# bupt-ai-cz/HIAST

Measured on AMD Instinct MI355X. Metric: self-training images/sec (fwd+bwd+pseudo-label) at 1024x512, higher is better.
Workload: dtype fp16

## Files before the change

### hiast_amd/_lib.py

```python
import ctypes
import os

import torch

_HERE = os.path.dirname(os.path.abspath(__file__))
LIB_PATH = os.environ.get("HIAST_LIB") or os.path.join(_HERE, "csrc", "libhiast_hip.so")

c_int, c_i64, c_f32, c_sz, c_vp = (ctypes.c_int, ctypes.c_int64, ctypes.c_float, ctypes.c_size_t,
                                   ctypes.c_void_p)

SIGNATURES = {
    "hiast_version": (c_int, []),
    "hiast_error_string": (ctypes.c_char_p, [c_int]),
    "hiast_upsample_bilinear_ac_fwd": (c_int, [c_vp, c_vp] + [c_int] * 6 + [c_vp]),
    "hiast_upsample_bilinear_ac_bwd": (c_int, [c_vp, c_vp] + [c_int] * 6 + [c_vp]),
    "hiast_plabel_pass1_workspace_bytes": (c_sz, [c_int]),
    "hiast_plabel_pass1": (c_int, [c_vp] + [c_int] * 6 + [c_vp, c_vp, c_vp, c_vp, c_sz, c_vp]),
    "hiast_plabel_pass2": (c_int, [c_vp, c_vp, c_vp, c_int, c_int, c_i64, c_vp, c_vp, c_vp, c_vp]),
    "hiast_plabel_strided_hist_workspace_bytes": (c_sz, [c_i64, c_int]),
    "hiast_plabel_strided_hist": (c_int, [c_vp, c_vp, c_i64, c_int, c_int, c_vp, c_vp, c_vp, c_vp, c_sz, c_vp]),
    "hiast_tta_fused": (c_int, [c_vp] * 6 + [c_int] * 5 + [c_vp, c_vp, c_vp]),
    "hiast_plabel_pass1_tta_workspace_bytes": (c_sz, [c_int]),
    "hiast_plabel_pass1_tta": (c_int, [c_vp] * 6 + [c_int] * 5 + [c_vp, c_vp, c_vp, c_vp, c_sz, c_vp]),
    "hiast_dinput_fwd": (c_int, [c_vp, c_int, c_vp] + [c_int] * 6 + [c_vp]),
# ... 41 lines not shown
    "hiast_conv_wgrad_nhwc": (c_int, [c_vp, c_vp, c_vp] + [c_int] * 9 + [c_vp, c_sz, c_vp]),
    "hiast_conv_wgrad_group_workspace_bytes": (c_sz, [c_vp, c_int]),
    "hiast_conv_wgrad_group_nhwc": (c_int, [c_vp, c_int, c_int, c_vp, c_sz, c_vp]),
    "hiast_conv_wgrad_small_workspace_bytes": (c_sz, [c_int] * 6),
    "hiast_conv_wgrad_small_nhwc": (c_int, [c_vp, c_vp, c_vp] + [c_int] * 9 + [c_vp, c_sz, c_vp]),
    "hiast_pack_conv_weight": (c_int, [c_vp, c_int, c_int, c_int, c_int, c_int, c_vp, c_vp, c_vp]),
    "hiast_bn_nhwc_workspace_bytes": (c_sz, [c_int]),
    "hiast_bn_nhwc_stats": (c_int, [c_vp, c_i64, c_int, c_vp, c_vp, c_sz, c_int, c_vp]),
    "hiast_bn_nhwc_apply": (c_int, [c_vp] * 8 + [ctypes.c_double, c_f32, c_f32, c_int, c_vp, c_vp, c_i64, c_int, c_vp,
                                    c_int, c_vp]),
    "hiast_bn_nhwc_apply_partial": (c_int, [c_vp] * 8 + [c_int, ctypes.c_double, c_f32, c_f32, c_int, c_vp, c_vp, c_i64,
                                            c_int, c_vp, c_int, c_vp]),
    "hiast_bn_nhwc_bwd_stats": (c_int, [c_vp] * 7 + [c_int, c_i64, c_int, c_vp, c_vp, c_sz, c_int, c_vp]),
    "hiast_bn_nhwc_bwd_apply": (c_int, [c_vp] * 8 + [ctypes.c_double, c_int, c_vp, c_vp, c_vp, c_vp, c_i64, c_int, c_int,
                                        c_vp]),
    "hiast_pack_conv_weight_multi": (c_int, [c_vp, c_vp, c_vp, c_int, c_int, c_vp]),
    "hiast_split_planes": (c_int, [c_vp, c_vp, c_i64, c_int, c_int, c_vp]),
    "hiast_stem_tail": (c_int, [c_vp, c_int, c_vp, c_vp, c_vp, c_vp, c_f32, c_vp, c_int, c_int, c_int, c_int, c_int, c_vp]),
    "hiast_stem_eval": (c_int, [c_vp] * 6 + [c_f32, c_vp, c_int, c_int, c_int, c_int, c_vp]),
    "hiast_stem_train_blocks": (c_int, [c_int] * 3),
    "hiast_stem_train_fwd": (c_int, [c_vp, c_vp, c_vp, c_vp, c_int, c_int, c_int, c_int, c_vp]),
    "hiast_stem_wgrad_workspace_bytes": (c_sz, [c_int] * 3),
    "hiast_stem_wgrad": (c_int, [c_vp, c_vp, c_vp, c_int, c_int, c_int, c_int, c_vp, c_sz, c_vp]),
    "hiast_ema_update": (c_int, [c_vp, c_vp, c_vp, c_int, c_f32, c_f32, c_vp]),
    "hiast_normalize_u8": (c_int, [c_vp, c_vp, c_int, c_i64, c_vp, c_vp, c_vp]),
    "hiast_maxpool3x3s2_nhwc_fwd": (c_int, [c_vp, c_vp, c_vp, c_int, c_int, c_int, c_int, c_int, c_vp]),
    "hiast_maxpool3x3s2_nhwc_bwd": (c_int, [c_vp, c_vp, c_vp, c_int, c_int, c_int, c_int, c_int, c_vp]),
    "hiast_multi_copy": (c_int, [c_vp, c_int, c_vp]),
    "hiast_aug_geometry_u8": (c_int, [c_vp] * 6 + [c_int] * 4 + [c_vp]),
    "hiast_aug_hist_u8": (c_int, [c_vp] * 5 + [c_int, c_i64, c_vp]),
# ... 77 lines not shown
```

### hiast_amd/csrc/bn_nhwc.hip

```cpp
#include <hip/hip_bf16.h>

#include "common.h"

namespace hiast {

constexpr int BNH_MAXBLK = 512;
#ifndef BNH_ROWS_PER_BLOCK_PASS
#define BNH_ROWS_PER_BLOCK_PASS 16
#endif
#ifndef BNH_APPLY_MAXBLK
#define BNH_APPLY_MAXBLK 65535
#endif
#ifndef BNH_CONTIG
#define BNH_CONTIG 0
#endif
#if BNH_CONTIG
#define BNH_ROW_WALK(CHUNK)                                                                                              \
    const long long step = (CHUNK);                                                                                      \
    const long long per_blk = ((M + gridDim.x - 1) / gridDim.x + (CHUNK) - 1) / (CHUNK) * (CHUNK);                       \
    const long long lim = (long long)(blockIdx.x + 1) * per_blk < M ? (long long)(blockIdx.x + 1) * per_blk : M;         \
    long long r0 = (long long)blockIdx.x * per_blk + rsub;
#else
#define BNH_ROW_WALK(CHUNK)                                                                                              \
    const long long step = (long long)gridDim.x * (CHUNK);                                                               \
// ... 194 lines not shown
    if (c >= C) return;
    const double m = sums[2 * c] / count;
    double var = sums[2 * c + 1] / count - m * m;
    var = var < 0.0 ? 0.0 : var;
    const float mean = (float)m;
    const float invstd = (float)(1.0 / sqrt(var + (double)eps));
    save_mean[c] = mean;
    save_invstd[c] = invstd;
    if (run_mean) {
        const double unb = count > 1.0 ? var * count / (count - 1.0) : var;
        run_mean[c] = (1.0f - momentum) * run_mean[c] + momentum * mean;
        run_var[c] = (1.0f - momentum) * run_var[c] + momentum * (float)unb;
    }
}

__global__ __launch_bounds__(256) void bnh_finalize_prep_kernel(const float* __restrict__ partial, int nblk, int C,
                                                                double count, float momentum, float eps,
                                                                float* __restrict__ run_mean, float* __restrict__ run_var,
                                                                float* __restrict__ save_mean,
                                                                float* __restrict__ save_invstd)
{
    __shared__ double s[64][5];
    const int e = threadIdx.x & 3, j = threadIdx.x >> 2;
    const int i = blockIdx.x * 4 + e;
    const int c = blockIdx.x * 2 + (int)threadIdx.x;
    float rm = 0.f, rv = 0.f;
    if (threadIdx.x < 2 && run_mean) { rm = run_mean[c]; rv = run_var[c]; }
    double acc = 0.0;
    {
        int b = j;
        for (; b + 64 * 3 < nblk; b += 64 * 4) {
            float v[4];
#pragma unroll
            for (int u = 0; u < 4; ++u) v[u] = partial[(size_t)(b + 64 * u) * C * 2 + i];
#pragma unroll
            for (int u = 0; u < 4; ++u) acc += (double)v[u];
        }
// ... 7 lines not shown
        for (int q = 0; q < 64; ++q) { s1 += s[q][2 * threadIdx.x]; s2 += s[q][2 * threadIdx.x + 1]; }
        const double m = s1 / count;
        double var = s2 / count - m * m;
        var = var < 0.0 ? 0.0 : var;
        const float mean = (float)m;
        save_mean[c] = mean;
        save_invstd[c] = (float)(1.0 / sqrt(var + (double)eps));
        if (run_mean) {
            const double unb = count > 1.0 ? var * count / (count - 1.0) : var;
            run_mean[c] = (1.0f - momentum) * rm + momentum * mean;
            run_var[c] = (1.0f - momentum) * rv + momentum * (float)unb;
        }
    }
}

template <bool RES, bool RELU, bool F16 = false>
__global__ __launch_bounds__(256) void bnh_apply_kernel(const unsigned short* __restrict__ x,
                                                        const unsigned short* __restrict__ res,
                                                        unsigned short* __restrict__ y, const float* __restrict__ gamma,
                                                        const float* __restrict__ beta,
                                                        const float* __restrict__ save_mean,
                                                        const float* __restrict__ save_invstd, long long M, int C,
                                                        unsigned char* __restrict__ mask)
{
    const int G = C >> 3, RPP = 256 / G;
    const bool nt_out = (long long)M * C * 2 >= H_NT_MIN_BYTES;
    const int cg = threadIdx.x % G, rsub = threadIdx.x / G;
    constexpr int UNR = BNH_UNR_APPLY;
    const long long stride = RPP;
    BNH_ROW_WALK(RPP * UNR)
// ... 108 lines not shown
            float g[8], yy[8], xx[8];
            bnh_unpack8<F16>(rg[u], g);
            if (GATE == 1) bnh_unpack8<F16>(ry[u], yy);
            const unsigned bits = rbits[u];
            bnh_unpack8<F16>(rx[u], xx);
#pragma unroll
            for (int k = 0; k < 8; ++k) {
                const bool open = GATE == 0 || (GATE == 1 ? yy[k] > 0.f
                                                : (GATE == 3 ? ((bits >> k) & 1u) != 0u : fmaf(xx[k], k0[k], gsh[k]) > 0.f));
                const float gg = open ? g[k] : 0.f;
                g[k] = gg;
                xx[k] = k0[k] * (gg - mg[k] - (xx[k] - mean[k]) * invstd[k] * mgx[k]);
            }
            bnh_store8<F16>(dx + off, xx, nt_out);
            if (DRES) bnh_store8<F16>(dres + off, g, nt_out);
        }
        r0 += step;
        if (r0 < lim) load_rows(r0);
    }
}

static int bnh_nblk(long long M, int C)
{
    const int rpp = 256 / (C / 8);
    long long nb = (M + (long long)rpp * 16 - 1) / ((long long)rpp * 16);
    nb = nb < 1 ? 1 : (nb > BNH_MAXBLK ? BNH_MAXBLK : nb);
    return (int)nb;
}

}
// ... 159 lines not shown
#define L1(G, DRES, F)                                                                                             \
    hipLaunchKernelGGL((hiast::bnh_bwd_apply_kernel<G, DRES, F>), dim3((unsigned)nb), dim3(256), 0, st,             \
                       (const unsigned short*)dy, (const unsigned short*)y, (const unsigned short*)x, gamma, beta,  \
                       save_mean, save_invstd, sums, 1.0 / count, (unsigned short*)dx, (unsigned short*)dres, dgamma, \
                       dbeta, (long long)M, C)
#define L(G, DRES) do { if (f16) L1(G, DRES, true); else L1(G, DRES, false); } while (0)
    if (relu == 1) { if (dres) L(1, true); else L(1, false); }
    else if (relu == 3) { if (dres) L(3, true); else L(3, false); }
    else if (relu == 2) { if (dres) L(2, true); else L(2, false); }
    else { if (dres) L(0, true); else L(0, false); }
#undef L
#undef L1
    HIAST_CHECK_LAUNCH();
    return 0;
}
```

### hiast_amd/functional.py

```python
import os

import torch

from . import kernels as K
from . import switches as SW

ASPP_DILATIONS = (6, 12, 18, 24)
H16 = (torch.bfloat16, torch.float16)


class _AsppFn(torch.autograd.Function):

    @staticmethod
    @torch.amp.custom_fwd(device_type="cuda", cast_inputs=torch.float32)
    def forward(ctx, x, w0, w1, w2, w3, b0, b1, b2, b3, dil):
        x = x.contiguous()
        ws = [w.contiguous() for w in (w0, w1, w2, w3)]
        bs = [b.contiguous() for b in (b0, b1, b2, b3)]
        wpack = K.aspp_pack_weights(ws, bs)
        Cout = ws[0].shape[0]
        y = K.aspp_fwd(x, wpack, Cout, dil)
        ctx.save_for_backward(x, wpack)
        ctx.dil = dil
        ctx.cin = x.shape[1]
# ... 309 lines not shown
        else:
            if fused is not None:
                sums = K.bn_nhwc_stats_from_partial(fused)
            else:
                sums = K.bn_nhwc_bwd_stats(dy, y, x, gamma, beta, sm, si, ctx.gate)
            if ctx.world != 1:
                _stat_all_reduce(sums)
        want_p = gamma is not None and (ctx.needs_input_grad[2] or ctx.needs_input_grad[3])
        handoff = ctx.box is not None and ctx.needs_input_grad[1]
        dx, dres, dg, db = K.bn_nhwc_bwd_apply(dy, y, x, gamma, beta, sm, si, sums, ctx.count, ctx.gate,
                                               ctx.has_res and ctx.needs_input_grad[1] and not handoff, want_p)
        if handoff:
            ctx.box["gated"] = (dy, y)
        return (dx, dres, dg if ctx.needs_input_grad[2] else None, db if ctx.needs_input_grad[3] else None,
                None, None, None, None, None, None, None, None, None)


class _ConvNhwcFn(torch.autograd.Function):

    @staticmethod
    @torch.amp.custom_fwd(device_type="cuda")
    def forward(ctx, x, weight, stride, dil, want_stats, box, packed, in_bn=None, wgroup=None, xsum=None, in_bn3=None):
        xv = x.permute(0, 2, 3, 1)
        ctx.in_bn3 = None
        if (in_bn3 is not None and "bn3" in in_bn3 and box is not None and stride == 1 and weight.shape[2] == 1
                and ctx.needs_input_grad[0] and _BN3_FUSION
                and K.xconv_dgrad_gated_bn_stats_ok(x.shape[0] * x.shape[2] * x.shape[3], weight.shape[0], weight.shape[1])):
            ctx.in_bn3 = in_bn3
        ctx.wgroup = wgroup
        ctx.xsum = xsum if (xsum is not None and stride == 1 and ctx.needs_input_grad[0]) else None
# ... 453 lines not shown

_nbt_batched = [False]


def bn_act(x, bn, res=None, relu=True, partial=None, box=None, stat_box=None):
    training = bn.training or (bn.running_mean is None)
    if training and bn.track_running_stats and bn.num_batches_tracked is not None and not _nbt_batched[0]:
        bn.num_batches_tracked.add_(1)
    momentum = 0.1 if bn.momentum is None else bn.momentum
    if (training and x.dtype in H16 and _is_cl(x) and not x.is_contiguous()
            and K.bn_nhwc_supported(x.shape[1]) and (res is None or (res.dtype == x.dtype and _is_cl(res)))):
        return _BnActNhwcFn.apply(x, res, bn.weight, bn.bias, bn.running_mean, bn.running_var, momentum, bn.eps, relu,
                                  _sync_world(bn), partial, box, stat_box)
    return _BnActFn.apply(x, res, bn.weight, bn.bias, bn.running_mean, bn.running_var, training, momentum,
                          bn.eps, relu, _sync_world(bn) if training else 1)
```

### hiast_amd/kernels.py

```python
import ctypes

import numpy as np
import torch

from . import _lib
from . import switches as _SW
from ._lib import NBINS, check


def _stream():
    return ctypes.c_void_p(torch._C._cuda_getCurrentRawStream(torch._C._cuda_getDevice()))


def _ptr(t):
    return ctypes.c_void_p(t.data_ptr()) if t is not None else ctypes.c_void_p(0)


def h2d_async(host, device, out=None):
    stage = torch.from_numpy(np.ascontiguousarray(host)).pin_memory()
    if out is None:
        return stage.to(device, non_blocking=True)
    out.copy_(stage.view(out.dtype).reshape(out.shape) if stage.dtype != out.dtype else stage.reshape(out.shape),
              non_blocking=True)
    return out
# ... 1369 lines not shown


def bn_nhwc_supported(C):
    return 8 <= C <= 2048 and (C & (C - 1)) == 0


def bn_nhwc_stats(x):
    xv, M, C = _bnh_view(x, "x")
    sums = torch.empty((C, 2), dtype=torch.float64, device=x.device)
    ws = _bnh_workspace(C, x.device)
    check(_lib.load().hiast_bn_nhwc_stats(_ptr(xv), M, C, _ptr(sums), _ptr(ws), ws.numel() * 4, fmt_of(x), _stream()),
          "hiast_bn_nhwc_stats")
    return sums


def bn_nhwc_stats_from_partial(partial):
    _req(partial, torch.float32, 3, "partial")
    nblk, C, two = partial.shape
    assert two == 2
    sums = torch.empty((C, 2), dtype=torch.float64, device=partial.device)
    check(_lib.load().hiast_bn_nhwc_stats_from_partial(_ptr(partial), nblk, C, _ptr(sums), _stream()),
          "hiast_bn_nhwc_stats_from_partial")
    return sums


def bn_nhwc_apply(x, res, gamma, beta, running_mean, running_var, sums, count, momentum, eps, relu, want_mask=False):
    xv, M, C = _bnh_view(x, "x")
    y = torch.empty_like(x, memory_format=torch.channels_last)
    mask = torch.empty((M, C // 8), dtype=torch.uint8, device=x.device) if want_mask else None
    rv = None
    if res is not None:
        rv, M2, C2 = _bnh_view(res, "res")
        assert (M2, C2) == (M, C)
    assert sums.dtype == torch.float64 and tuple(sums.shape) == (C, 2) and sums.is_contiguous()
    sm = torch.empty(C, dtype=torch.float32, device=x.device)
# ... 36 lines not shown


def bn_nhwc_bwd_apply(dy, y, x, gamma, beta, save_mean, save_invstd, sums, count, gate, want_dres, want_dparam):
    xv, M, C = _bnh_view(x, "x")
    dv = _bnh_view(dy, "dy")[0]
    yv = _bnh_view(y, "y")[0] if gate == 1 else (_req(y, torch.uint8, 2, "mask") if gate == 3 else None)
    dx = torch.empty_like(x, memory_format=torch.channels_last)
    dres = torch.empty_like(x, memory_format=torch.channels_last) if want_dres else None
    dg = torch.empty(C, dtype=torch.float32, device=x.device) if want_dparam else None
    db = torch.empty(C, dtype=torch.float32, device=x.device) if want_dparam else None
    check(_lib.load().hiast_bn_nhwc_bwd_apply(_ptr(dv), _ptr(yv), _ptr(xv), _ptr(gamma), _ptr(beta), _ptr(save_mean),
                                              _ptr(save_invstd), _ptr(sums), float(count), int(gate), _ptr(dx),
                                              _ptr(dres), _ptr(dg), _ptr(db), M, C, fmt_of(x), _stream()),
          "hiast_bn_nhwc_bwd_apply")
    return dx, dres, dg, db


_wgrad_ws = {}


def conv_wgrad_supported(Cin, Cout, k, stride):
    return Cin % 256 == 0 and Cout % 256 == 0 and k in (1, 3) and (k == 3 or stride == 1)


def conv_wgrad_preferred(Cin, Cout, k, stride):
    import os
    if not conv_wgrad_supported(Cin, Cout, k, stride):
        return False
    return k == 1 or os.environ.get("HIAST_LIB_WGRAD3", "0") != "1"

# ... 211 lines not shown
```

### hiast_amd/sseg/models/modules/resnet.py

```python
import os

import torch
import torch.nn as nn
import torch.nn.functional as F

from hiast_amd import functional as HF


def bn_act(bn, x, res=None, relu=True, partial=None):
    if x.is_cuda:
        return HF.bn_act(x, bn, res, relu, partial=partial)
    y = bn(x)
    if res is not None:
        y = y + res
    return F.relu(y) if relu else y


def conv(m, x):
    if x.is_cuda and x.dtype in HF.H16 and HF.conv_nhwc_ok(x, m):
        return HF.conv_nhwc(x, m)
    return m(x)


def conv_bn_act(cv, bn, x, res=None, relu=True, conv_box=None, bn_box=None, in_bn=None, stat_box=None, wgroup=None, xsum=None,
                in_bn3=None):
    if x.is_cuda and x.dtype in HF.H16 and bn.training and HF.conv_nhwc_ok(x, cv):
        y, partial = HF.conv_nhwc(x, cv, want_stats=True, box=conv_box, in_bn=in_bn, wgroup=wgroup, xsum=xsum, in_bn3=in_bn3)
        return HF.bn_act(y, bn, res, relu, partial=partial, box=bn_box, stat_box=stat_box)
    return bn_act(bn, conv(cv, x), res, relu)


def _nhwc2d(t):
    B, C, H, W = t.shape
    return t.permute(0, 2, 3, 1).reshape(B * H * W, C)


def _from2d(y2d, B, H, W):
    return y2d.view(B, H, W, y2d.shape[1]).permute(0, 3, 1, 2)


def packed_weight(conv, fmt):
    from hiast_amd import kernels as K
    w = conv.weight
# ... 13 lines not shown
        super().__init__()
        self.conv1 = nn.Conv2d(inplanes, planes, 1, bias=False)
        self.bn1 = nn.BatchNorm2d(planes)
        self.conv2 = nn.Conv2d(planes, planes, 3, stride=stride, padding=dilation, dilation=dilation, bias=False)
        self.bn2 = nn.BatchNorm2d(planes)
        self.conv3 = nn.Conv2d(planes, planes * 4, 1, bias=False)
        self.bn3 = nn.BatchNorm2d(planes * 4)
        self.relu = nn.ReLU(inplace=True)
        self.downsample = downsample

    def forward(self, x):
        xs = None
        if (self.downsample is not None and self.downsample[0].stride == (1, 1) and x.is_cuda and x.dtype in HF.H16
                and self.bn1.training and x.requires_grad and not HF.SW.on("HIAST_NO_XSUM")):
            xs = {}
        idt = x if self.downsample is None else conv_bn_act(self.downsample[0], self.downsample[1], x, relu=False,
                                                            xsum=None if xs is None else (xs, "take"))
        box = {} if (self.downsample is None and not HF.SW.on("HIAST_NO_IDT_HANDOFF")) else None
        sb1, sb2 = {}, {}
        grp, wv = (None, None)
        if x.is_cuda and x.dtype in HF.H16 and self.bn1.training:
            grp, wv = HF.wgroup_weights((self.conv1, self.conv2, self.conv3), x)
        g = (lambda i: (grp, grp["slot"][i], wv[i]) if wv[i] is not None else None) if grp is not None else (lambda i: None)
        o = conv_bn_act(self.conv1, self.bn1, x, conv_box=box, stat_box=sb1, wgroup=g(0),
                        xsum=None if xs is None else (xs, "give"), in_bn3=getattr(x, "_hiast_bn3", None) if box is not None else None)
        o = conv_bn_act(self.conv2, self.bn2, o, in_bn=sb1, stat_box=sb2, wgroup=g(1))
        sb3 = {}
        y = conv_bn_act(self.conv3, self.bn3, o, res=idt, bn_box=box, in_bn=sb2, stat_box=sb3, wgroup=g(2))
        if "bn3" in sb3:
            y._hiast_bn3 = sb3
        return y

    def forward_eval_planes(self, x, fmt):
        from hiast_amd import kernels as K
        PL = 2 if fmt == K.FMT_SPLIT_BF16 else 1
        o = K.igemm_bn_act(x, packed_weight(self.conv1, fmt), PL, self.bn1, None, True)
        if self.downsample is None:
            idt = x
        else:
            dconv, dbn = self.downsample[0], self.downsample[1]
            xs = x if dconv.stride == (1, 1) else x[:, ::dconv.stride[0], ::dconv.stride[1]].contiguous()
            idt = K.igemm_bn_act(xs, packed_weight(dconv, fmt), PL, dbn, None, False)
        o = K.igemm_bn_act(o, packed_weight(self.conv2, fmt), PL, self.bn2, None, True, self.conv2.stride[0],
# ... 160 lines not shown
```

### hiast_amd/switches.py

```python
import os

_NAMES = ("HIAST_NO_BN_MASK", "HIAST_NO_BN_BWD_FUSION", "HIAST_LIB_WGRAD", "HIAST_NO_WGROUP", "HIAST_NO_XSUM",
          "HIAST_NO_IDT_HANDOFF", "HIAST_LIB_STEM")
SWITCHES = {n: os.environ.get(n, "0") == "1" for n in _NAMES}
_OPT_IN_NAMES = ("HIAST_DISC_HIP", "HIAST_DISC_HIP_16BIT")
OPT_IN = {n: os.environ.get(n, "0") == "1" for n in _OPT_IN_NAMES}


def on(name):
    return OPT_IN[name] if name in OPT_IN else SWITCHES[name]
```

### include/hiast_hip.h

```cpp
#ifndef HIAST_HIP_H
#define HIAST_HIP_H

#include <stddef.h>
#include <stdint.h>

#ifdef __cplusplus
extern "C" {
#endif

#define HIAST_ABI_VERSION 6

#define HIAST_E_ARG   (-1)
#define HIAST_E_RANGE (-2)
#define HIAST_E_WS    (-3)

#define HIAST_NBINS 15361
#define HIAST_PROB_FX_SHIFT 30
#define HIAST_MAX_CLASSES 32
#define HIAST_FMT_BF16 1
#define HIAST_FMT_SPLIT_BF16 2
#define HIAST_FMT_FP16 3
#define HIAST_IGNORE 255

typedef void* hiast_stream_t;
// ... 163 lines not shown
                                float* running_mean, float* running_var, const float* partial, int nblk, double count,
                                float momentum, float eps, int relu, float* save_mean, float* save_invstd, int64_t M,
                                int C, void* mask, int fmt, hiast_stream_t stream);
int hiast_bn_nhwc_apply(const void* x, const void* res, void* y, const float* gamma, const float* beta,
                        float* running_mean, float* running_var, const double* sums, double count, float momentum,
                        float eps, int relu, float* save_mean, float* save_invstd, int64_t M, int C, void* mask, int fmt,
                        hiast_stream_t stream);
int hiast_bn_nhwc_bwd_stats(const void* dy, const void* y, const void* x, const float* gamma, const float* beta,
                            const float* save_mean, const float* save_invstd, int relu, int64_t M, int C, double* sums,
                            void* workspace, size_t workspace_bytes, int fmt, hiast_stream_t stream);
int hiast_bn_nhwc_bwd_apply(const void* dy, const void* y, const void* x, const float* gamma, const float* beta,
                            const float* save_mean, const float* save_invstd, const double* sums, double count, int relu,
                            void* dx, void* dres, float* dgamma, float* dbeta, int64_t M, int C, int fmt,
                            hiast_stream_t stream);

typedef struct { float* ema; const float* p; int64_t n; } hiast_ema_rec;
int hiast_ema_update(const hiast_ema_rec* table, const int32_t* chunk_tensor,
                     const int64_t* chunk_start, int n_chunks, float gamma,
                     float one_minus_gamma, hiast_stream_t stream);

int hiast_maxpool3x3s2_nhwc_fwd(const void* x, void* y, uint8_t* idx, int B, int H, int W, int C,
                                int fmt , hiast_stream_t stream);
int hiast_maxpool3x3s2_nhwc_bwd(const void* dy, const uint8_t* idx, void* dx, int B, int H, int W, int C, int fmt,
                                hiast_stream_t stream);

int hiast_normalize_u8(const uint8_t* img, float* out, int B, int64_t HW, const float* mean, const float* std,
                       hiast_stream_t stream);

#define HIAST_AUG_REC_WORDS 20
#define HIAST_AUG_MAX_OPS 8
// ... 76 lines not shown
```

Baseline: 144.7.

## Fuse downsample BN and bn3 BN+residual+ReLU into dual-BN kernels

In ResNet bottleneck blocks that have a downsample branch, the downsample conv output is no longer normalized into a separate tensor. A new dual kernel applies both BatchNorms, adds the residual and ReLU in one pass, with matching fused backward stats and apply kernels. The two finalize steps also share one launch. This removes writing and re-reading the normalized identity tensor and several launches per block. The cost is more complex kernels with higher register pressure, and the identity is rounded to 16-bit inside the kernel to match the old numerics.

```diff
diff --git a/hiast_amd/_lib.py b/hiast_amd/_lib.py
--- a/hiast_amd/_lib.py
+++ b/hiast_amd/_lib.py
@@ -79,6 +79,10 @@
     "hiast_bn_nhwc_bwd_stats": (c_int, [c_vp] * 7 + [c_int, c_i64, c_int, c_vp, c_vp, c_sz, c_int, c_vp]),
     "hiast_bn_nhwc_bwd_apply": (c_int, [c_vp] * 8 + [ctypes.c_double, c_int, c_vp, c_vp, c_vp, c_vp, c_i64, c_int, c_int,
                                         c_vp]),
+    "hiast_bn_nhwc_dual_apply_partial": (c_int, [c_vp] * 8 + [c_int, c_f32, c_f32, c_vp, c_vp] + [c_vp] * 5 +
+                                         [c_int, c_f32, c_f32, c_vp, c_vp, ctypes.c_double, c_i64, c_int, c_vp, c_int, c_vp]),
+    "hiast_bn_nhwc_dual_bwd_stats": (c_int, [c_vp] * 8 + [c_i64, c_int, c_vp, c_vp, c_sz, c_int, c_vp]),
+    "hiast_bn_nhwc_dual_bwd_apply": (c_int, [c_vp] * 11 + [ctypes.c_double] + [c_vp] * 6 + [c_i64, c_int, c_int, c_vp]),
     "hiast_pack_conv_weight_multi": (c_int, [c_vp, c_vp, c_vp, c_int, c_int, c_vp]),
     "hiast_split_planes": (c_int, [c_vp, c_vp, c_i64, c_int, c_int, c_vp]),
     "hiast_stem_tail": (c_int, [c_vp, c_int, c_vp, c_vp, c_vp, c_vp, c_f32, c_vp, c_int, c_int, c_int, c_int, c_int, c_vp]),
diff --git a/hiast_amd/csrc/bn_nhwc.hip b/hiast_amd/csrc/bn_nhwc.hip
--- a/hiast_amd/csrc/bn_nhwc.hip
+++ b/hiast_amd/csrc/bn_nhwc.hip
@@ -232,13 +232,11 @@
     }
 }
 
-__global__ __launch_bounds__(256) void bnh_finalize_prep_kernel(const float* __restrict__ partial, int nblk, int C,
-                                                                double count, float momentum, float eps,
-                                                                float* __restrict__ run_mean, float* __restrict__ run_var,
-                                                                float* __restrict__ save_mean,
-                                                                float* __restrict__ save_invstd)
-{
-    __shared__ double s[64][5];
+__device__ __forceinline__ void bnh_finalize_prep_block(const float* __restrict__ partial, int nblk, int C, double count,
+                                                        float momentum, float eps, float* __restrict__ run_mean,
+                                                        float* __restrict__ run_var, float* __restrict__ save_mean,
+                                                        float* __restrict__ save_invstd, double (&s)[64][5])
+{
     const int e = threadIdx.x & 3, j = threadIdx.x >> 2;
     const int i = blockIdx.x * 4 + e;
     const int c = blockIdx.x * 2 + (int)threadIdx.x;
@@ -276,6 +274,31 @@
     }
 }
 
+__global__ __launch_bounds__(256) void bnh_finalize_prep_kernel(const float* __restrict__ partial, int nblk, int C,
+                                                                double count, float momentum, float eps,
+                                                                float* __restrict__ run_mean, float* __restrict__ run_var,
+                                                                float* __restrict__ save_mean,
+                                                                float* __restrict__ save_invstd)
+{
+    __shared__ double s[64][5];
+    bnh_finalize_prep_block(partial, nblk, C, count, momentum, eps, run_mean, run_var, save_mean, save_invstd, s);
+}
+
+struct BnhPrepSet {
+    const float* partial;
+    int nblk;
+    float momentum, eps;
+    float *run_mean, *run_var, *save_mean, *save_invstd;
+};
+
+__global__ __launch_bounds__(256) void bnh_finalize_prep2_kernel(BnhPrepSet a, BnhPrepSet b, int C, double count)
+{
+    __shared__ double s[64][5];
+    const BnhPrepSet p = blockIdx.y ? b : a;
+    bnh_finalize_prep_block(p.partial, p.nblk, C, count, p.momentum, p.eps, p.run_mean, p.run_var, p.save_mean,
+                            p.save_invstd, s);
+}
+
 template <bool RES, bool RELU, bool F16 = false>
 __global__ __launch_bounds__(256) void bnh_apply_kernel(const unsigned short* __restrict__ x,
                                                         const unsigned short* __restrict__ res,
@@ -414,6 +437,247 @@
             }
             bnh_store8<F16>(dx + off, xx, nt_out);
             if (DRES) bnh_store8<F16>(dres + off, g, nt_out);
+        }
+        r0 += step;
+        if (r0 < lim) load_rows(r0);
+    }
+}
+
+template <bool F16>
+__global__ __launch_bounds__(256) void bnh_apply_dual_kernel(
+    const unsigned short* __restrict__ x3, const unsigned short* __restrict__ xd, unsigned short* __restrict__ y,
+    const float* __restrict__ gamma3, const float* __restrict__ beta3, const float* __restrict__ save_mean3,
+    const float* __restrict__ save_invstd3, const float* __restrict__ gammad, const float* __restrict__ betad,
+    const float* __restrict__ save_meand, const float* __restrict__ save_invstdd, long long M, int C,
+    unsigned char* __restrict__ mask)
+{
+    const int G = C >> 3, RPP = 256 / G;
+    const bool nt_out = (long long)M * C * 2 >= H_NT_MIN_BYTES;
+    const int cg = threadIdx.x % G, rsub = threadIdx.x / G;
+    constexpr int UNR = BNH_UNR_APPLY;
+    const long long stride = RPP;
+    BNH_ROW_WALK(RPP * UNR)
+
+    uint4 r3[UNR], rd[UNR];
+    auto load_rows = [&](long long rb) {
+#pragma unroll
+        for (int u = 0; u < UNR; ++u) {
+            const long long r = rb + u * stride;
+            const size_t off = (size_t)(r < lim ? r : (rb < lim ? rb : 0)) * C + cg * 8;
+            r3[u] = bnh_ld16<1>(x3 + off);
+            rd[u] = bnh_ld16<1>(xd + off);
+        }
+    };
+    load_rows(r0);
+    float scale3[8], shift3[8], scaled[8], shiftd[8];
+    {
+        float gm[8], bt[8], mn[8], is[8];
+        bnh_param8(gamma3, save_mean3, cg * 8, 1.0f, gm);
+        bnh_param8(beta3, save_mean3, cg * 8, 0.0f, bt);
+        bnh_param8(save_mean3, save_mean3, cg * 8, 0.f, mn);
+        bnh_param8(save_invstd3, save_mean3, cg * 8, 0.f, is);
+#pragma unroll
+        for (int k = 0; k < 8; ++k) {
+            scale3[k] = gm[k] * is[k];
+            shift3[k] = fmaf(-mn[k], scale3[k], bt[k]);
+        }
+        bnh_param8(gammad, save_meand, cg * 8, 1.0f, gm);
+        bnh_param8(betad, save_meand, cg * 8, 0.0f, bt);
+        bnh_param8(save_meand, save_meand, cg * 8, 0.f, mn);
+        bnh_param8(save_invstdd, save_meand, cg * 8, 0.f, is);
+#pragma unroll
+        for (int k = 0; k < 8; ++k) {
+            scaled[k] = gm[k] * is[k];
+            shiftd[k] = fmaf(-mn[k], scaled[k], bt[k]);
+        }
+    }
+    while (r0 < lim) {
+#pragma unroll
+        for (int u = 0; u < UNR; ++u) {
+            const long long r = r0 + u * stride;
+            if (r >= lim) break;
+            const size_t off = (size_t)r * C + cg * 8;
+            float v[8], rr[8];
+            bnh_unpack8<F16>(r3[u], v);
+            bnh_unpack8<F16>(rd[u], rr);
+#pragma unroll
+            for (int k = 0; k < 8; ++k) {
+                rr[k] = fmaf(rr[k], scaled[k], shiftd[k]);
+                asm volatile("" : "+v"(rr[k]));
+            }
+            const uint4 rq = make_uint4(H16<F16>::pack(rr[0], rr[1]), H16<F16>::pack(rr[2], rr[3]),
+                                        H16<F16>::pack(rr[4], rr[5]), H16<F16>::pack(rr[6], rr[7]));
+            bnh_unpack8<F16>(rq, rr);
+            unsigned bits = 0;
+#pragma unroll
+            for (int k = 0; k < 8; ++k) {
+                float o = fmaf(v[k], scale3[k], shift3[k]);
+                o += rr[k];
+                o = o > 0.f ? o : 0.f;
+                bits |= (o > 0.f ? 1u : 0u) << k;
+                v[k] = o;
+            }
+            bnh_store8<F16>(y + off, v, nt_out);
+            if (mask) mask[(size_t)r * G + cg] = (unsigned char)bits;
+        }
+        r0 += step;
+        if (r0 < lim) load_rows(r0);
+    }
+}
+
+template <bool F16>
+__global__ __launch_bounds__(256) void bnh_partial_dual_kernel(
+    const unsigned short* __restrict__ dy, const unsigned char* __restrict__ mask, const unsigned short* __restrict__ x3,
+    const unsigned short* __restrict__ xd, const float* __restrict__ save_mean3, const float* __restrict__ save_invstd3,
+    const float* __restrict__ save_meand, const float* __restrict__ save_invstdd, long long M, int C,
+    float* __restrict__ partial)
+{
+    __shared__ float s_red[256 * 16];
+    const int G = C >> 3, RPP = 256 / G;
+    const int cg = threadIdx.x % G, rsub = threadIdx.x / G;
+    float s1[8], s23[8], s2d[8], mean3[8], invstd3[8], meand[8], invstdd[8];
+#pragma unroll
+    for (int k = 0; k < 8; ++k) { s1[k] = 0.f; s23[k] = 0.f; s2d[k] = 0.f; }
+    constexpr int UNR = BNH_UNR_PART;
+    const long long stride = RPP;
+    BNH_ROW_WALK(RPP * UNR)
+
+    uint4 rg[UNR], r3[UNR], rd[UNR];
+    unsigned rbits[UNR];
+    auto load_rows = [&](long long rb) {
+#pragma unroll
+        for (int u = 0; u < UNR; ++u) {
+            const long long r = rb + u * stride;
+            const long long rc = r < lim ? r : (rb < lim ? rb : 0);
+            const size_t off = (size_t)rc * C + cg * 8;
+            rg[u] = bnh_ld16<0>(dy + off);
+            rbits[u] = mask[(size_t)rc * G + cg];
+            r3[u] = bnh_ld16<0>(x3 + off);
+            rd[u] = bnh_ld16<0>(xd + off);
+        }
+    };
+    load_rows(r0);
+    bnh_param8(save_mean3, save_mean3, cg * 8, 0.f, mean3);
+    bnh_param8(save_invstd3, save_mean3, cg * 8, 0.f, invstd3);
+    bnh_param8(save_meand, save_meand, cg * 8, 0.f, meand);
+    bnh_param8(save_invstdd, save_meand, cg * 8, 0.f, invstdd);
+    while (r0 < lim) {
+#pragma unroll
+        for (int u = 0; u < UNR; ++u) {
+            if (r0 + u * stride >= lim) break;
+            float v[8], a[8], b[8];
+            bnh_unpack8<F16>(rg[u], v);
+            const unsigned bits = rbits[u];
+            bnh_unpack8<F16>(r3[u], a);
+            bnh_unpack8<F16>(rd[u], b);
+#pragma unroll
+            for (int k = 0; k < 8; ++k) {
+                const float g = ((bits >> k) & 1u) != 0u ? v[k] : 0.f;
+                s1[k] += g;
+                s23[k] = fmaf(g, (a[k] - mean3[k]) * invstd3[k], s23[k]);
+                s2d[k] = fmaf(g, (b[k] - meand[k]) * invstdd[k], s2d[k]);
+            }
+        }
+        r0 += step;
+        if (r0 < lim) load_rows(r0);
+    }
+#pragma unroll
+    for (int set = 0; set < 2; ++set) {
+        if (set) __syncthreads();
+#pragma unroll
+        for (int k = 0; k < 8; ++k) {
+            s_red[threadIdx.x * 16 + k] = s1[k];
+            s_red[threadIdx.x * 16 + 8 + k] = set ? s2d[k] : s23[k];
+        }
+        __syncthreads();
+        if (rsub == 0) {
+            float* dst = partial + ((size_t)blockIdx.x * 2 * C + (size_t)set * C + cg * 8) * 2;
+#pragma unroll
+            for (int k = 0; k < 8; ++k) {
+                float t1 = 0.f, t2 = 0.f;
+                for (int j = 0; j < RPP; ++j) {
+                    t1 += s_red[(j * G + cg) * 16 + k];
+                    t2 += s_red[(j * G + cg) * 16 + 8 + k];
+                }
+                dst[2 * k] = t1;
+                dst[2 * k + 1] = t2;
+            }
+        }
+    }
+}
+
+template <bool F16>
+__global__ __launch_bounds__(256) void bnh_bwd_apply_dual_kernel(
+    const unsigned short* __restrict__ dy, const unsigned char* __restrict__ mask, const unsigned short* __restrict__ x3,
+    const unsigned short* __restrict__ xd, const float* __restrict__ gamma3, const float* __restrict__ save_mean3,
+    const float* __restrict__ save_invstd3, const double* __restrict__ sums3, const float* __restrict__ gammad,
+    const float* __restrict__ save_meand, const float* __restrict__ save_invstdd, const double* __restrict__ sumsd,
+    double inv_count, unsigned short* __restrict__ dx3, unsigned short* __restrict__ dxd, float* __restrict__ dgamma3,
+    float* __restrict__ dbeta3, float* __restrict__ dgammad, float* __restrict__ dbetad, long long M, int C)
+{
+    const int G = C >> 3, RPP = 256 / G;
+    const bool nt_out = (long long)M * C * 2 >= H_NT_MIN_BYTES;
+    const int cg = threadIdx.x % G, rsub = threadIdx.x / G;
+    constexpr int UNR = BNH_UNR_BWD;
+    const long long stride = RPP;
+    BNH_ROW_WALK(RPP * UNR)
+
+    uint4 rg[UNR], r3[UNR], rd[UNR];
+    unsigned rbits[UNR];
+    auto load_rows = [&](long long rb) {
+#pragma unroll
+        for (int u = 0; u < UNR; ++u) {
+            const long long r = rb + u * stride;
+            const long long rc = r < lim ? r : (rb < lim ? rb : 0);
+            const size_t off = (size_t)rc * C + cg * 8;
+            rg[u] = bnh_ld16<2>(dy + off);
+            rbits[u] = mask[(size_t)rc * G + cg];
+            r3[u] = bnh_ld16<2>(x3 + off);
+            rd[u] = bnh_ld16<2>(xd + off);
+        }
+    };
+    load_rows(r0);
+    float mean3[8], invstd3[8], k03[8], mg3[8], mgx3[8], meand[8], invstdd[8], k0d[8], mgd[8], mgxd[8];
+    auto prep = [&](const float* gamma, const float* save_mean, const float* save_invstd, const double* sums, float* dgamma,
+                    float* dbeta, float (&mean)[8], float (&invstd)[8], float (&k0)[8], float (&mg)[8], float (&mgx)[8]) {
+        float gm[8];
+        bnh_param8(save_mean, save_mean, cg * 8, 0.f, mean);
+        bnh_param8(save_invstd, save_mean, cg * 8, 0.f, invstd);
+        bnh_param8(gamma, save_mean, cg * 8, 1.0f, gm);
+        const double2* sp = reinterpret_cast<const double2*>(sums) + cg * 8;
+#pragma unroll
+        for (int k = 0; k < 8; ++k) {
+            const double2 ss = sp[k];
+            if (blockIdx.x == 0 && rsub == 0) {
+                if (dbeta) dbeta[cg * 8 + k] = (float)ss.x;
+                if (dgamma) dgamma[cg * 8 + k] = (float)ss.y;
+            }
+            k0[k] = gm[k] * invstd[k];
+            mg[k] = (float)(ss.x * inv_count);
+            mgx[k] = (float)(ss.y * inv_count);
+        }
+    };
+    prep(gamma3, save_mean3, save_invstd3, sums3, dgamma3, dbeta3, mean3, invstd3, k03, mg3, mgx3);
+    prep(gammad, save_meand, save_invstdd, sumsd, dgammad, dbetad, meand, invstdd, k0d, mgd, mgxd);
+    while (r0 < lim) {
+#pragma unroll
+        for (int u = 0; u < UNR; ++u) {
+            const long long r = r0 + u * stride;
+            if (r >= lim) break;
+            const size_t off = (size_t)r * C + cg * 8;
+            float g[8], a[8], b[8];
+            bnh_unpack8<F16>(rg[u], g);
+            const unsigned bits = rbits[u];
+            bnh_unpack8<F16>(r3[u], a);
+            bnh_unpack8<F16>(rd[u], b);
+#pragma unroll
+            for (int k = 0; k < 8; ++k) {
+                const float gg = ((bits >> k) & 1u) != 0u ? g[k] : 0.f;
+                a[k] = k03[k] * (gg - mg3[k] - (a[k] - mean3[k]) * invstd3[k] * mgx3[k]);
+                b[k] = k0d[k] * (gg - mgd[k] - (b[k] - meand[k]) * invstdd[k] * mgxd[k]);
+            }
+            bnh_store8<F16>(dx3 + off, a, nt_out);
+            bnh_store8<F16>(dxd + off, b, nt_out);
         }
         r0 += step;
         if (r0 < lim) load_rows(r0);
@@ -603,3 +867,109 @@
     HIAST_CHECK_LAUNCH();
     return 0;
 }
+
+static long long bnh_apply_blocks(long long M, int C)
+{
+    const int rpp = 256 / (C / 8);
+    long long nb = (M + (long long)rpp * BNH_ROWS_PER_BLOCK_PASS - 1) / ((long long)rpp * BNH_ROWS_PER_BLOCK_PASS);
+    return nb < 1 ? 1 : (nb > BNH_APPLY_MAXBLK ? BNH_APPLY_MAXBLK : nb);
+}
+
+extern "C" int hiast_bn_nhwc_dual_apply_partial(
+    const void* x3, const void* xd, void* y, const float* gamma3, const float* beta3, float* running_mean3,
+    float* running_var3, const float* partial3, int nblk3, float momentum3, float eps3, float* save_mean3,
+    float* save_invstd3, const float* gammad, const float* betad, float* running_meand, float* running_vard,
+    const float* partiald, int nblkd, float momentumd, float epsd, float* save_meand, float* save_invstdd, double count,
+    int64_t M, int C, void* mask, int fmt, hiast_stream_t stream)
+{
+    BNH_FMT_CHECK();
+    int e = bnh_check(x3, M, C);
+    if (e) return e;
+    if (!xd || !y || !partial3 || !partiald || !save_mean3 || !save_invstd3 || !save_meand || !save_invstdd || count <= 0 ||
+        nblk3 <= 0 || nblkd <= 0 || (!running_mean3) != (!running_var3) || (!running_meand) != (!running_vard))
+        return HIAST_E_ARG;
+    if ((((uintptr_t)y) | ((uintptr_t)xd)) & 15) return HIAST_E_RANGE;
+    hipStream_t st = (hipStream_t)stream;
+    const hiast::BnhPrepSet s3 = {partial3, nblk3, momentum3, eps3, running_mean3, running_var3, save_mean3, save_invstd3};
+    const hiast::BnhPrepSet sd = {partiald, nblkd, momentumd, epsd, running_meand, running_vard, save_meand, save_invstdd};
+    hipLaunchKernelGGL(hiast::bnh_finalize_prep2_kernel, dim3(C / 2, 2), dim3(256), 0, st, s3, sd, C, count);
+    HIAST_CHECK_LAUNCH();
+    const unsigned nb = (unsigned)bnh_apply_blocks(M, C);
+#define L(F)                                                                                                           \
+    hipLaunchKernelGGL((hiast::bnh_apply_dual_kernel<F>), dim3(nb), dim3(256), 0, st, (const unsigned short*)x3,       \
+                       (const unsigned short*)xd, (unsigned short*)y, gamma3, beta3, save_mean3, save_invstd3, gammad, \
+                       betad, save_meand, save_invstdd, (long long)M, C, (unsigned char*)mask)
+    if (f16) L(true); else L(false);
+#undef L
+    HIAST_CHECK_LAUNCH();
+    return 0;
+}
+
+extern "C" int hiast_bn_nhwc_dual_bwd_stats(const void* dy, const void* mask, const void* x3, const void* xd,
+                                            const float* save_mean3, const float* save_invstd3, const float* save_meand,
+                                            const float* save_invstdd, int64_t M, int C, double* sums, void* workspace,
+                                            size_t workspace_bytes, int fmt, hiast_stream_t stream)
+{
+    BNH_FMT_CHECK();
+    int e = bnh_check(xd, M, C);
+    if (e) return e;
+    if (!dy || !mask || !save_meand || !save_invstdd || !sums || !workspace || (x3 && (!save_mean3 || !save_invstd3)))
+        return HIAST_E_ARG;
+    if ((((uintptr_t)dy) | ((uintptr_t)x3)) & 15) return HIAST_E_RANGE;
+    const int nblk = hiast::bnh_nblk(M, C);
+    hipStream_t st = (hipStream_t)stream;
+    if (!x3) {
+        if (workspace_bytes < (size_t)nblk * C * 2 * sizeof(float)) return HIAST_E_WS;
+#define L(F)                                                                                                           \
+    hipLaunchKernelGGL((hiast::bnh_partial_kernel<true, 3, F>), dim3(nblk), dim3(256), 0, st, (const unsigned short*)dy, \
+                       (const unsigned short*)mask, (const unsigned short*)xd, nullptr, nullptr, save_meand,           \
+                       save_invstdd, (long long)M, C, (float*)workspace)
+        if (f16) L(true); else L(false);
+#undef L
+        HIAST_CHECK_LAUNCH();
+        hipLaunchKernelGGL(hiast::bnh_finalize_kernel, dim3(C * 2 / 16), dim3(256), 0, st, (const float*)workspace, nblk, C,
+                           sums + (size_t)C * 2);
+        HIAST_CHECK_LAUNCH();
+        return 0;
+    }
+    if (workspace_bytes < (size_t)nblk * C * 4 * sizeof(float)) return HIAST_E_WS;
+#define L(F)                                                                                                           \
+    hipLaunchKernelGGL((hiast::bnh_partial_dual_kernel<F>), dim3(nblk), dim3(256), 0, st, (const unsigned short*)dy,   \
+                       (const unsigned char*)mask, (const unsigned short*)x3, (const unsigned short*)xd, save_mean3,   \
+                       save_invstd3, save_meand, save_invstdd, (long long)M, C, (float*)workspace)
+    if (f16) L(true); else L(false);
+#undef L
+    HIAST_CHECK_LAUNCH();
+    hipLaunchKernelGGL(hiast::bnh_finalize_kernel, dim3(C * 4 / 16), dim3(256), 0, st, (const float*)workspace, nblk, 2 * C,
+                       sums);
+    HIAST_CHECK_LAUNCH();
+    return 0;
+}
+
+extern "C" int hiast_bn_nhwc_dual_bwd_apply(const void* dy, const void* mask, const void* x3, const void* xd,
+                                            const float* gamma3, const float* save_mean3, const float* save_invstd3,
+                                            const float* gammad, const float* save_meand, const float* save_invstdd,
+                                            const double* sums, double count, void* dx3, void* dxd, float* dgamma3,
+                                            float* dbeta3, float* dgammad, float* dbetad, int64_t M, int C, int fmt,
+                                            hiast_stream_t stream)
+{
+    BNH_FMT_CHECK();
+    int e = bnh_check(x3, M, C);
+    if (e) return e;
+    if (!dy || !mask || !xd || !save_mean3 || !save_invstd3 || !save_meand || !save_invstdd || !sums || !dx3 || !dxd ||
+        count <= 0)
+        return HIAST_E_ARG;
+    if ((((uintptr_t)dy) | ((uintptr_t)xd) | ((uintptr_t)dx3) | ((uintptr_t)dxd)) & 15) return HIAST_E_RANGE;
+    const unsigned nb = (unsigned)bnh_apply_blocks(M, C);
+    hipStream_t st = (hipStream_t)stream;
+#define L(F)                                                                                                           \
+    hipLaunchKernelGGL((hiast::bnh_bwd_apply_dual_kernel<F>), dim3(nb), dim3(256), 0, st, (const unsigned short*)dy,   \
+                       (const unsigned char*)mask, (const unsigned short*)x3, (const unsigned short*)xd, gamma3,       \
+                       save_mean3, save_invstd3, sums, gammad, save_meand, save_invstdd, sums + (size_t)C * 2,         \
+                       1.0 / count, (unsigned short*)dx3, (unsigned short*)dxd, dgamma3, dbeta3, dgammad, dbetad,      \
+                       (long long)M, C)
+    if (f16) L(true); else L(false);
+#undef L
+    HIAST_CHECK_LAUNCH();
+    return 0;
+}
diff --git a/hiast_amd/functional.py b/hiast_amd/functional.py
--- a/hiast_amd/functional.py
+++ b/hiast_amd/functional.py
@@ -347,6 +347,48 @@
             ctx.box["gated"] = (dy, y)
         return (dx, dres, dg if ctx.needs_input_grad[2] else None, db if ctx.needs_input_grad[3] else None,
                 None, None, None, None, None, None, None, None, None)
+
+
+class _BnDualNhwcFn(torch.autograd.Function):
+
+    @staticmethod
+    def forward(ctx, x3, xd, gamma3, beta3, gammad, betad, bn3, bnd, partial3, partiald, stat_box):
+        count = float(x3.shape[0] * x3.shape[2] * x3.shape[3])
+        y, st3, std, mask = K.bn_nhwc_dual_apply_partial(x3, xd, (gamma3, beta3) + bn3, (gammad, betad) + bnd, partial3,
+                                                         partiald, count)
+        ctx.save_for_backward(x3, xd, mask, gamma3, gammad, st3[0], st3[1], std[0], std[1])
+        ctx.count = count
+        ctx.stat_box = None
+        if stat_box is not None:
+            left = stat_box.pop("bwd_sums", None)
+            if left is not None:
+                _stat_wait(left[1])
+            stat_box.pop("bwd_partial", None)
+            stat_box["bn3"] = (x3.detach(), mask, st3[0], st3[1])
+            stat_box["world"] = 1
+            ctx.stat_box = stat_box
+        return y
+
+    @staticmethod
+    def backward(ctx, dy):
+        x3, xd, mask, gamma3, gammad, sm3, si3, smd, sid = ctx.saved_tensors
+        if dy.dtype != x3.dtype:
+            dy = dy.to(x3.dtype)
+        dy = dy.contiguous(memory_format=torch.channels_last)
+        fused = ctx.stat_box.pop("bwd_partial", None) if ctx.stat_box is not None else None
+        if fused is not None:
+            C = x3.shape[1]
+            sums = torch.empty((2, C, 2), dtype=torch.float64, device=x3.device)
+            K.bn_nhwc_stats_from_partial(fused, out=sums[0])
+            K.bn_nhwc_dual_bwd_stats(dy, mask, None, xd, None, (smd, sid), sums=sums)
+        else:
+            sums = K.bn_nhwc_dual_bwd_stats(dy, mask, x3, xd, (sm3, si3), (smd, sid))
+        nig = ctx.needs_input_grad
+        dx3, dxd, p3, pd = K.bn_nhwc_dual_bwd_apply(dy, mask, x3, xd, gamma3, (sm3, si3), gammad, (smd, sid), sums,
+                                                    ctx.count, gamma3 is not None and (nig[2] or nig[3]),
+                                                    gammad is not None and (nig[4] or nig[5]))
+        return (dx3, dxd, p3[0] if nig[2] else None, p3[1] if nig[3] else None, pd[0] if nig[4] else None,
+                pd[1] if nig[5] else None, None, None, None, None, None)
 
 
 class _ConvNhwcFn(torch.autograd.Function):
@@ -830,3 +872,26 @@
                                   _sync_world(bn), partial, box, stat_box)
     return _BnActFn.apply(x, res, bn.weight, bn.bias, bn.running_mean, bn.running_var, training, momentum,
                           bn.eps, relu, _sync_world(bn) if training else 1)
+
+
+def bn_dual_ok(bn3, bnd):
+    if SW.on("HIAST_NO_DUAL_BN") or SW.on("HIAST_NO_BN_MASK"):
+        return False
+    for bn in (bn3, bnd):
+        if not bn.training or _sync_world(bn) != 1:
+            return False
+    return bn3.num_features == bnd.num_features
+
+
+def bn_dual_act(x3, partial3, bn3, xd, partiald, bnd, stat_box=None):
+    ok = lambda t: (t.is_cuda and t.dtype in H16 and _is_cl(t) and not t.is_contiguous() and K.bn_nhwc_supported(t.shape[1]))
+    if not (ok(x3) and ok(xd) and x3.shape == xd.shape and x3.dtype == xd.dtype and partial3 is not None
+            and partiald is not None):
+        return bn_act(x3, bn3, bn_act(xd, bnd, None, False, partial=partiald), True, partial=partial3, stat_box=stat_box)
+    args = []
+    for bn in (bn3, bnd):
+        if bn.track_running_stats and bn.num_batches_tracked is not None and not _nbt_batched[0]:
+            bn.num_batches_tracked.add_(1)
+        args.append((bn.running_mean, bn.running_var, 0.1 if bn.momentum is None else bn.momentum, bn.eps))
+    return _BnDualNhwcFn.apply(x3, xd, bn3.weight, bn3.bias, bnd.weight, bnd.bias, args[0], args[1], partial3, partiald,
+                               stat_box)
diff --git a/hiast_amd/kernels.py b/hiast_amd/kernels.py
--- a/hiast_amd/kernels.py
+++ b/hiast_amd/kernels.py
@@ -1407,11 +1407,12 @@
     return sums
 
 
-def bn_nhwc_stats_from_partial(partial):
+def bn_nhwc_stats_from_partial(partial, out=None):
     _req(partial, torch.float32, 3, "partial")
     nblk, C, two = partial.shape
     assert two == 2
-    sums = torch.empty((C, 2), dtype=torch.float64, device=partial.device)
+    sums = torch.empty((C, 2), dtype=torch.float64, device=partial.device) if out is None else _req(out, torch.float64, 2, "out")
+    assert tuple(sums.shape) == (C, 2)
     check(_lib.load().hiast_bn_nhwc_stats_from_partial(_ptr(partial), nblk, C, _ptr(sums), _stream()),
           "hiast_bn_nhwc_stats_from_partial")
     return sums
@@ -1478,6 +1479,64 @@
                                               _ptr(dres), _ptr(dg), _ptr(db), M, C, fmt_of(x), _stream()),
           "hiast_bn_nhwc_bwd_apply")
     return dx, dres, dg, db
+
+
+def bn_nhwc_dual_apply_partial(x3, xd, bn3, bnd, partial3, partiald, count, want_mask=True):
+    v3, M, C = _bnh_view(x3, "x3")
+    vd, M2, C2 = _bnh_view(xd, "xd")
+    assert (M2, C2) == (M, C) and xd.dtype == x3.dtype
+    for p in (partial3, partiald):
+        _req(p, torch.float32, 3, "partial")
+        assert p.shape[1] == C and p.shape[2] == 2
+    y = torch.empty_like(x3, memory_format=torch.channels_last)
+    mask = torch.empty((M, C // 8), dtype=torch.uint8, device=x3.device) if want_mask else None
+    sv = [torch.empty(C, dtype=torch.float32, device=x3.device) for _ in range(4)]
+    g3, b3, rm3, rv3, mom3, eps3 = bn3
+    gd, bd, rmd, rvd, momd, epsd = bnd
+    check(_lib.load().hiast_bn_nhwc_dual_apply_partial(
+        _ptr(v3), _ptr(vd), _ptr(y), _ptr(g3), _ptr(b3), _ptr(rm3), _ptr(rv3), _ptr(partial3), partial3.shape[0],
+        float(mom3), float(eps3), _ptr(sv[0]), _ptr(sv[1]), _ptr(gd), _ptr(bd), _ptr(rmd), _ptr(rvd), _ptr(partiald),
+        partiald.shape[0], float(momd), float(epsd), _ptr(sv[2]), _ptr(sv[3]), float(count), M, C, _ptr(mask), fmt_of(x3),
+        _stream()), "hiast_bn_nhwc_dual_apply_partial")
+    return y, (sv[0], sv[1]), (sv[2], sv[3]), mask
+
+
+def bn_nhwc_dual_bwd_stats(dy, mask, x3, xd, stat3, statd, sums=None):
+    vd, M, C = _bnh_view(xd, "xd")
+    dv, M2, C2 = _bnh_view(dy, "dy")
+    assert (M2, C2) == (M, C)
+    v3 = None
+    if x3 is not None:
+        v3, M3, C3 = _bnh_view(x3, "x3")
+        assert (M3, C3) == (M, C)
+    _req(mask, torch.uint8, 2, "mask")
+    assert tuple(mask.shape) == (M, C // 8)
+    if sums is None:
+        sums = torch.empty((2, C, 2), dtype=torch.float64, device=xd.device)
+    assert sums.dtype == torch.float64 and tuple(sums.shape) == (2, C, 2) and sums.is_contiguous()
+    ws = _bnh_workspace(2 * C, xd.device)
+    sm3, si3 = stat3 if x3 is not None else (None, None)
+    check(_lib.load().hiast_bn_nhwc_dual_bwd_stats(_ptr(dv), _ptr(mask), _ptr(v3), _ptr(vd), _ptr(sm3), _ptr(si3),
+                                                   _ptr(statd[0]), _ptr(statd[1]), M, C, _ptr(sums), _ptr(ws),
+                                                   ws.numel() * 4, fmt_of(xd), _stream()), "hiast_bn_nhwc_dual_bwd_stats")
+    return sums
+
+
+def bn_nhwc_dual_bwd_apply(dy, mask, x3, xd, gamma3, stat3, gammad, statd, sums, count, want_dparam3, want_dparamd):
+    v3, M, C = _bnh_view(x3, "x3")
+    vd = _bnh_view(xd, "xd")[0]
+    dv = _bnh_view(dy, "dy")[0]
+    _req(mask, torch.uint8, 2, "mask")
+    assert sums.dtype == torch.float64 and tuple(sums.shape) == (2, C, 2) and sums.is_contiguous()
+    dx3 = torch.empty_like(x3, memory_format=torch.channels_last)
+    dxd = torch.empty_like(xd, memory_format=torch.channels_last)
+    new = lambda want: torch.empty(C, dtype=torch.float32, device=x3.device) if want else None
+    dg3, db3, dgd, dbd = new(want_dparam3), new(want_dparam3), new(want_dparamd), new(want_dparamd)
+    check(_lib.load().hiast_bn_nhwc_dual_bwd_apply(_ptr(dv), _ptr(mask), _ptr(v3), _ptr(vd), _ptr(gamma3), _ptr(stat3[0]),
+                                                   _ptr(stat3[1]), _ptr(gammad), _ptr(statd[0]), _ptr(statd[1]), _ptr(sums),
+                                                   float(count), _ptr(dx3), _ptr(dxd), _ptr(dg3), _ptr(db3), _ptr(dgd),
+                                                   _ptr(dbd), M, C, fmt_of(x3), _stream()), "hiast_bn_nhwc_dual_bwd_apply")
+    return dx3, dxd, (dg3, db3), (dgd, dbd)
 
 
 _wgrad_ws = {}
diff --git a/hiast_amd/sseg/models/modules/resnet.py b/hiast_amd/sseg/models/modules/resnet.py
--- a/hiast_amd/sseg/models/modules/resnet.py
+++ b/hiast_amd/sseg/models/modules/resnet.py
@@ -23,10 +23,14 @@
 
 
 def conv_bn_act(cv, bn, x, res=None, relu=True, conv_box=None, bn_box=None, in_bn=None, stat_box=None, wgroup=None, xsum=None,
-                in_bn3=None):
+                in_bn3=None, dual=None):
     if x.is_cuda and x.dtype in HF.H16 and bn.training and HF.conv_nhwc_ok(x, cv):
         y, partial = HF.conv_nhwc(x, cv, want_stats=True, box=conv_box, in_bn=in_bn, wgroup=wgroup, xsum=xsum, in_bn3=in_bn3)
+        if dual is not None:
+            return HF.bn_dual_act(y, partial, bn, dual[0], dual[1], dual[2], stat_box=stat_box)
         return HF.bn_act(y, bn, res, relu, partial=partial, box=bn_box, stat_box=stat_box)
+    if dual is not None:
+        res = HF.bn_act(dual[0], dual[2], None, False, partial=dual[1])
     return bn_act(bn, conv(cv, x), res, relu)
 
 
@@ -70,8 +74,14 @@
         if (self.downsample is not None and self.downsample[0].stride == (1, 1) and x.is_cuda and x.dtype in HF.H16
                 and self.bn1.training and x.requires_grad and not HF.SW.on("HIAST_NO_XSUM")):
             xs = {}
-        idt = x if self.downsample is None else conv_bn_act(self.downsample[0], self.downsample[1], x, relu=False,
-                                                            xsum=None if xs is None else (xs, "take"))
+        dual = None
+        if (self.downsample is not None and x.is_cuda and x.dtype in HF.H16 and HF.conv_nhwc_ok(x, self.downsample[0])
+                and HF.bn_dual_ok(self.bn3, self.downsample[1])):
+            dual = HF.conv_nhwc(x, self.downsample[0], want_stats=True, xsum=None if xs is None else (xs, "take"))
+            idt = None
+        else:
+            idt = x if self.downsample is None else conv_bn_act(self.downsample[0], self.downsample[1], x, relu=False,
+                                                                xsum=None if xs is None else (xs, "take"))
         box = {} if (self.downsample is None and not HF.SW.on("HIAST_NO_IDT_HANDOFF")) else None
         sb1, sb2 = {}, {}
         grp, wv = (None, None)
@@ -82,7 +92,8 @@
                         xsum=None if xs is None else (xs, "give"), in_bn3=getattr(x, "_hiast_bn3", None) if box is not None else None)
         o = conv_bn_act(self.conv2, self.bn2, o, in_bn=sb1, stat_box=sb2, wgroup=g(1))
         sb3 = {}
-        y = conv_bn_act(self.conv3, self.bn3, o, res=idt, bn_box=box, in_bn=sb2, stat_box=sb3, wgroup=g(2))
+        y = conv_bn_act(self.conv3, self.bn3, o, res=idt, bn_box=box, in_bn=sb2, stat_box=sb3, wgroup=g(2),
+                        dual=None if dual is None else (dual[0], dual[1], self.downsample[1]))
         if "bn3" in sb3:
             y._hiast_bn3 = sb3
         return y
diff --git a/hiast_amd/switches.py b/hiast_amd/switches.py
--- a/hiast_amd/switches.py
+++ b/hiast_amd/switches.py
@@ -5,7 +5,11 @@
 SWITCHES = {n: os.environ.get(n, "0") == "1" for n in _NAMES}
 _OPT_IN_NAMES = ("HIAST_DISC_HIP", "HIAST_DISC_HIP_16BIT")
 OPT_IN = {n: os.environ.get(n, "0") == "1" for n in _OPT_IN_NAMES}
+_FUSED_OFF_NAMES = ("HIAST_NO_DUAL_BN",)
+FUSED_OFF = {n: os.environ.get(n, "0") == "1" for n in _FUSED_OFF_NAMES}
 
 
 def on(name):
+    if name in FUSED_OFF:
+        return FUSED_OFF[name]
     return OPT_IN[name] if name in OPT_IN else SWITCHES[name]
diff --git a/include/hiast_hip.h b/include/hiast_hip.h
--- a/include/hiast_hip.h
+++ b/include/hiast_hip.h
@@ -201,6 +201,23 @@
                             void* dx, void* dres, float* dgamma, float* dbeta, int64_t M, int C, int fmt,
                             hiast_stream_t stream);
 
+int hiast_bn_nhwc_dual_apply_partial(const void* x3, const void* xd, void* y, const float* gamma3, const float* beta3,
+                                     float* running_mean3, float* running_var3, const float* partial3, int nblk3,
+                                     float momentum3, float eps3, float* save_mean3, float* save_invstd3,
+                                     const float* gammad, const float* betad, float* running_meand, float* running_vard,
+                                     const float* partiald, int nblkd, float momentumd, float epsd, float* save_meand,
+                                     float* save_invstdd, double count, int64_t M, int C, void* mask, int fmt,
+                                     hiast_stream_t stream);
+int hiast_bn_nhwc_dual_bwd_stats(const void* dy, const void* mask, const void* x3, const void* xd,
+                                 const float* save_mean3, const float* save_invstd3, const float* save_meand,
+                                 const float* save_invstdd, int64_t M, int C, double* sums, void* workspace,
+                                 size_t workspace_bytes, int fmt, hiast_stream_t stream);
+int hiast_bn_nhwc_dual_bwd_apply(const void* dy, const void* mask, const void* x3, const void* xd, const float* gamma3,
+                                 const float* save_mean3, const float* save_invstd3, const float* gammad,
+                                 const float* save_meand, const float* save_invstdd, const double* sums, double count,
+                                 void* dx3, void* dxd, float* dgamma3, float* dbeta3, float* dgammad, float* dbetad,
+                                 int64_t M, int C, int fmt, hiast_stream_t stream);
+
 typedef struct { float* ema; const float* p; int64_t n; } hiast_ema_rec;
 int hiast_ema_update(const hiast_ema_rec* table, const int32_t* chunk_tensor,
                      const int64_t* chunk_start, int n_chunks, float gamma,
```

Result: no change. 144.6 (-0.1%).
